# MaxInGaussian/SCFGP

Measured on AMD Instinct MI355X. Metric: NLML+grad evals/sec, higher is better.
Workload: dtype f32

## Files before the change

scfgp_amd/csrc/gram.hip:

```cpp
#include "kernels.h"
#include "tile_cfgs.h"

#include <algorithm>

#ifdef SCFGP_TRACE
constexpr int TRACE_CAP = 1 << 16;
__device__ unsigned long long g_trace[TRACE_CAP][4];
#define TRACE_BEGIN() const unsigned long long tr_t0 = __builtin_amdgcn_s_memrealtime()
#define TRACE_END(kind)                                                                                     \
    do {                                                                                                    \
        __syncthreads();                                                                                    \
        if (threadIdx.x == 0 && j < TRACE_CAP) {                                                            \
            g_trace[j][0] = tr_t0; g_trace[j][1] = __builtin_amdgcn_s_memrealtime();                        \
            g_trace[j][2] = (unsigned long long)__builtin_amdgcn_s_getreg((20 << 0) | (0 << 6) | (3 << 11)) |             \
                            ((unsigned long long)__builtin_amdgcn_s_getreg((4 << 0) | (0 << 6) | (31 << 11)) << 8);       \
            g_trace[j][3] = (unsigned long long)(kind);                                                     \
        }                                                                                                   \
    } while (0)
int64_t trace_read(void* host, int64_t max_bytes) {
    const int64_t n = max_bytes < (int64_t)sizeof(g_trace) ? max_bytes : (int64_t)sizeof(g_trace);
    return hipMemcpyFromSymbol(host, HIP_SYMBOL(g_trace), n) == hipSuccess ? n : -2;
}
#else
#define TRACE_BEGIN()
// ... 69 lines not shown
    double* __restrict__ slab, double* __restrict__ slab_hi, char* smem_raw) {
    if (diag) gram_body_impl<Cfg, WEIGHT, STRIP, true>(Phi, ld, w, side, r0, r1, chunk, acol, bcol, sideout, slab, slab_hi, smem_raw);
    else gram_body_impl<Cfg, WEIGHT, STRIP, false>(Phi, ld, w, side, r0, r1, chunk, acol, bcol, sideout, slab, slab_hi, smem_raw);
}

struct GramDma {
    static constexpr int BM = 256, BN = 128, A_BYTES = 16 * BM * 4, B_BYTES = 16 * BN * 4, W_OFF = A_BYTES + B_BYTES,
                         STAGE = W_OFF + 256, STAGES = 3, LDS_BYTES = STAGES * STAGE, DMA_PER_WAVE = (A_BYTES + B_BYTES) / 1024 / 8;
    static_assert(DMA_PER_WAVE == 3, "8 waves, 24 KiB of operands per stage");
};
typedef __attribute__((address_space(3))) void lds_void;
typedef const __attribute__((address_space(1))) void gbl_void;
__device__ __forceinline__ lds_void* lds_ptr(const char* p) { return (lds_void*)(uintptr_t)((unsigned)(uintptr_t)p); }
struct GramDmaWide {
    static constexpr int BM = 64, BN = 512, A_BYTES = 16 * BM * 4, B_BYTES = 16 * BN * 4, W_OFF = A_BYTES + B_BYTES,
                         STAGE = W_OFF + 256, STAGES = 2, LDS_BYTES = STAGES * STAGE, NINSTR = (A_BYTES + B_BYTES) / 1024, DMA_PER_WAVE = 5;
    static_assert(NINSTR == 36 && 2 * LDS_BYTES <= 160 * 1024, "two workgroups per CU");
};
struct GramDmaSq {
    static constexpr int BM = 128, BN = 128, A_BYTES = 16 * BM * 4, B_BYTES = 16 * BN * 4, W_OFF = A_BYTES + B_BYTES,
                         STAGE = W_OFF + 256, STAGES = 3, LDS_BYTES = STAGES * STAGE, DMA_PER_WAVE = (A_BYTES + B_BYTES) / 1024 / 8;
    static_assert(DMA_PER_WAVE == 2, "8 waves, 16 KiB of operands per stage");
};
struct GramDmaPair {
    static constexpr int BM = 256, BN = 128, A_BYTES = 16 * BM * 4, B_BYTES = 0, W_OFF = A_BYTES,
                         STAGE = W_OFF + 256, STAGES = 3, LDS_BYTES = STAGES * STAGE, DMA_PER_WAVE = A_BYTES / 1024 / 8;
    static_assert(DMA_PER_WAVE == 2, "8 waves, 16 KiB of operands per stage");
};
template <class D, bool WEIGHT, bool DIAG, bool TRANS = false>
__device__ __forceinline__ void gram_pipe_dma(
    const float* __restrict__ Phi, int64_t ld, const float* __restrict__ ws2,
    int64_t r0, int64_t r1, int64_t chunk, int acol, int bcol, double* __restrict__ sideout,
    double* __restrict__ slab, double* __restrict__ slab_hi, char* smem) {
    constexpr bool WIDE = D::BM == 64, SQ = D::BM == 128, PAIR = D::B_BYTES == 0;
    constexpr int RING = D::STAGES, TM = SQ ? 2 : 4;
    typedef std::integral_constant<int, 0> H0;
    typedef std::integral_constant<int, 1> H1;
    constexpr bool WS = WEIGHT || DIAG;
    constexpr int DPW = D::DMA_PER_WAVE, NRD = 4 + (WEIGHT || DIAG ? 2 : 0), NM = 8 * TM, PRE = 2;
    static_assert(PRE + DPW + 1 + NRD <= NM, "one fetch or read per MFMA behind the barrier");
    static_assert(!(PAIR && DIAG), "the paired diagonal blocks carry no side sums");
    static_assert(!TRANS || (D::BM == 256 && D::B_BYTES != 0 && !DIAG), "transposed flush: off-diagonal tall tiles");
    int tid = threadIdx.x;
    asm volatile("" : "+v"(tid));
    const int lane = tid & 63, wave = __builtin_amdgcn_readfirstlane(tid >> 6), i = lane & 15, q = lane >> 4;
    const int wm0 = WIDE ? 0 : (wave >> 1) * (16 * TM), wn0 = WIDE ? wave * 64 : (wave & 1) * 64;
    const char* src[DPW]; int dst[DPW];
#pragma unroll
    for (int u = 0; u < DPW; ++u) {
        const int t = WIDE ? wave + 8 * u : DPW * wave + u;
        const float* g;
        if constexpr (PAIR) g = Phi + (r0 + t) * ld + (lane < 32 ? acol : bcol - 128) + 4 * lane;
        else if constexpr (SQ) g = t < 8 ? Phi + (r0 + 2 * t + (lane >> 5)) * ld + acol + ((4 * (lane & 31) - 32 * (lane >> 5)) & 127)
                                    : Phi + (r0 + 2 * (t - 8) + (lane >> 5)) * ld + bcol + 4 * (lane & 31);
        else if constexpr (WIDE) g = t < 4 ? Phi + (r0 + 4 * t + (lane >> 4)) * ld + acol + 4 * (lane & 15) : Phi + (r0 + ((t - 4) >> 1)) * ld + bcol + 256 * ((t - 4) & 1) + 4 * lane;
        else g = t < 16 ? Phi + (r0 + t) * ld + acol + 4 * lane : Phi + (r0 + 2 * (t - 16) + (lane >> 5)) * ld + bcol + 4 * (lane & 31);
        src[u] = reinterpret_cast<const char*>(g);
        dst[u] = t * 1024;
    }
    const bool last_u = !WIDE || wave < 4;
    const int64_t step = 16 * ld * (int64_t)sizeof(float);
    const char* wsrc = WS ? reinterpret_cast<const char*>(ws2 + 2 * r0) + 4 * lane : nullptr;
    const bool ws_wave = WS && wave == 0;
    const auto fetch_one = [&](auto uc, int slot) {
        constexpr int u = decltype(uc)::value;
        char* base = smem + slot * D::STAGE;
        if constexpr (u < DPW) {
            if (u < DPW - 1 || last_u) {
                __builtin_amdgcn_global_load_lds((gbl_void*)src[u], lds_ptr(base + dst[u]), 16, 0, 0);
                src[u] += step;
            }
        } else if (ws_wave) {
            __builtin_amdgcn_global_load_lds((gbl_void*)wsrc, lds_ptr(base + D::W_OFF), 4, 0, 0);
            wsrc += 128;
        }
    };
    const int ring = (int)(uintptr_t)smem;
    const int pa0 = SQ ? ring + q * (D::BM * 4) + ((wm0 + 2 * i + 32 * (q & 1)) & 127) * 4 : ring + q * (D::BM * 4) + (wm0 + 4 * i) * 4, pb0 = PAIR ? ring + q * (D::BM * 4) + ((wm0 & 128) + wn0 + 4 * i) * 4 : ring + D::A_BYTES + q * (D::BN * 4) + (wn0 + 4 * i) * 4, pw0 = ring + D::W_OFF + q * 8;
    typedef float v2f __attribute__((ext_vector_type(2)));
    typedef float afrag_t __attribute__((ext_vector_type(TM)));
    afrag_t fa[2][2]; v4f fb[2][2];
    v2f fws[2][2];
    v4f acc[TM][4];
    afrag_t sacc = 0.f;
    const auto read_one = [&](auto hc, auto rc, int stage) {
        constexpr int h = decltype(hc)::value, R = decltype(rc)::value, kk = 2 * h + (R & 1);
        (void)&fws; (void)&pw0; (void)&fa; (void)&fb; (void)&pa0; (void)&pb0;
        if constexpr (R < 2 && SQ) asm volatile("ds_read_b64 %0, %1 offset:%2" : "=v"(fa[h][R & 1]) : "v"(stage + pa0), "n"(kk * 4 * D::BM * 4));
        else if constexpr (R < 2) asm volatile("ds_read_b128 %0, %1 offset:%2" : "=v"(fa[h][R & 1]) : "v"(stage + pa0), "n"(kk * 4 * D::BM * 4));
        else if constexpr (R < 4) asm volatile("ds_read_b128 %0, %1 offset:%2" : "=v"(fb[h][R & 1]) : "v"(stage + pb0), "n"(kk * 4 * (PAIR ? D::BM : D::BN) * 4));
        else asm volatile("ds_read_b64 %0, %1 offset:%2" : "=v"(fws[h][R & 1]) : "v"(stage + pw0), "n"(kk * 32));
    };
#define SCFGP_WAIT_FRAGS(what, h)                                                                                                        \
    do {                                                                                                                                 \
        if constexpr (WS)                                                                                                                \
            asm volatile("s_waitcnt " what : "+v"(fa[h][0]), "+v"(fa[h][1]), "+v"(fb[h][0]), "+v"(fb[h][1]), "+v"(fws[h][0]), "+v"(fws[h][1]) :: "memory"); \
        else asm volatile("s_waitcnt " what : "+v"(fa[h][0]), "+v"(fa[h][1]), "+v"(fb[h][0]), "+v"(fb[h][1]) :: "memory");              \
        __builtin_amdgcn_sched_barrier(0);                                                                                               \
        if constexpr (DIAG) { sacc += fws[h][0][1] * fa[h][0]; sacc += fws[h][1][1] * fa[h][1]; }        \
        if constexpr (WEIGHT) { fa[h][0] *= fws[h][0][0]; fa[h][1] *= fws[h][1][0]; }                                                    \
        __builtin_amdgcn_sched_barrier(0);                                                                                               \
    } while (0)
    const auto mfma_one = [&](auto hc, auto ic) {
        constexpr int h = decltype(hc)::value, I = decltype(ic)::value, k2 = I / (4 * TM), tm = I / 4 % TM, tn = I % 4;
        acc[tm][tn] = __builtin_amdgcn_mfma_f32_16x16x4f32(fa[h][k2][tm], fb[h][k2][tn], acc[tm][tn], 0, 0, 0);
        __builtin_amdgcn_sched_barrier(0);
    };
    const auto second_half_pre = [&]() { static_for<PRE>([&](auto ic) { mfma_one(H1(), ic); }); };
    const auto second_half = [&](auto fc, auto rdc, int fslot, int next) {
        static_for<NM - PRE>([&](auto ic) {
            constexpr int I = decltype(ic)::value;
            mfma_one(H1(), std::integral_constant<int, I + PRE>());
            if constexpr (I < DPW + 1) {
                if constexpr (decltype(fc)::value && (I < DPW || WS)) { fetch_one(ic, fslot); __builtin_amdgcn_sched_barrier(0); }
            } else if constexpr (I - DPW - 1 < NRD) {
                if constexpr (decltype(rdc)::value) { read_one(H0(), std::integral_constant<int, I - DPW - 1>(), next); __builtin_amdgcn_sched_barrier(0); }
            }
        });
    };
    const auto first_half = [&](int next) {
        static_for<NM>([&](auto ic) {
            mfma_one(H0(), ic);
            if constexpr (decltype(ic)::value < NRD) { read_one(H1(), ic, next); __builtin_amdgcn_sched_barrier(0); }
        });
    };
    double* sl = TRANS ? (wm0 >= 128 ? slab_hi : slab) + (int64_t)wn0 * 128 + (wm0 & 127)
               : WIDE  ? slab + (int64_t)(wn0 >> 7) * (128 * 128) + (wn0 & 127)
                       : (wm0 >= 128 ? slab_hi + (int64_t)(wm0 - 128) * 128 : slab + (int64_t)wm0 * 128) + wn0;
    bool first = true;
    const auto flush = [&]() {
        int lf = lane;
        asm volatile("" : "+v"(lf));
        const int i = lf & 15, q = lf >> 4;
        if constexpr (TRANS) {
#pragma unroll
            for (int tn = 0; tn < 4; ++tn)
#pragma unroll
                for (int r = 0; r < 4; ++r) {
                    v4d* d = reinterpret_cast<v4d*>(sl + (4 * i + tn) * 128 + 4 * (4 * q + r));
                    const v4d v = v4d{(double)acc[0][tn][r], (double)acc[1][tn][r], (double)acc[2][tn][r], (double)acc[3][tn][r]};
                    *d = first ? v : *d + v;
                }
        } else {
#pragma unroll
        for (int tm = 0; tm < TM; ++tm)
#pragma unroll
            for (int r = 0; r < 4; ++r) {
                v4d* d = reinterpret_cast<v4d*>(sl + (TM * (4 * q + r) + tm) * 128 + 4 * i);
                const v4d v = v4d{(double)acc[tm][0][r], (double)acc[tm][1][r], (double)acc[tm][2][r], (double)acc[tm][3][r]};
                *d = first ? v : *d + v;
            }
        }
        if constexpr (DIAG) {
#pragma unroll
            for (int tm = 0; tm < TM; ++tm) {
                double x = (double)sacc[tm];
                x += __shfl_xor(x, 16); x += __shfl_xor(x, 32);
                if (q == 0 && wn0 == 0) { double* d = sideout + wm0 + TM * i + tm; *d = first ? x : *d + x; }
            }
            sacc = 0.f;
        }
#pragma unroll
        for (int tm = 0; tm < TM; ++tm)
#pragma unroll
            for (int tn = 0; tn < 4; ++tn) acc[tm][tn] = v4f{0.f, 0.f, 0.f, 0.f};
        first = false;
    };
#pragma unroll
    for (int tm = 0; tm < TM; ++tm)
#pragma unroll
        for (int tn = 0; tn < 4; ++tn) acc[tm][tn] = v4f{0.f, 0.f, 0.f, 0.f};
    const auto strip_rest = [&]() {
        if constexpr (WIDE)
            for (int e = tid; e < 4 * 64 * 128; e += 512) slab[(e / (64 * 128)) * (128 * 128) + 64 * 128 + e % (64 * 128)] = 0.0;
    };
    const int nst = (int)((r1 - r0) / 16), per_chunk = (int)(chunk / 16);
    if (nst == 0) { flush(); strip_rest(); return; }
    static_for<DPW + 1>([&](auto uc) { fetch_one(uc, 0); });
    if (RING == 3 && nst > 1) static_for<DPW + 1>([&](auto uc) { fetch_one(uc, 1); });
    const auto wait_landed = [&](bool more) {
        if (RING == 3 && more) {
            if (ws_wave) asm volatile("s_waitcnt vmcnt(%0)" :: "n"(DPW + 1) : "memory"); else asm volatile("s_waitcnt vmcnt(%0)" :: "n"(DPW) : "memory");
        }
        else asm volatile("s_waitcnt vmcnt(0)" ::: "memory");
    };
    const auto next_slot = [&](int sl_) { return sl_ == RING - 1 ? 0 : sl_ + 1; };
    int slot = 0, s = 0;
    while (s < nst) {
        const int cend = s + per_chunk < nst ? s + per_chunk : nst;
        wait_landed(s + 1 < nst);
        __builtin_amdgcn_s_barrier();
        asm volatile("" ::: "memory");
        if (s + RING - 1 < nst) { const int fslot = slot == 0 ? RING - 1 : slot - 1; static_for<DPW + 1>([&](auto uc) { fetch_one(uc, fslot); }); }
        static_for<NRD>([&](auto rc) { read_one(H0(), rc, slot * D::STAGE); });
        static_for<NRD>([&](auto rc) { read_one(H1(), rc, slot * D::STAGE); });
        SCFGP_WAIT_FRAGS("lgkmcnt(0)", 0);
        static_for<NM>([&](auto ic) { mfma_one(H0(), ic); });
// ... 103 lines not shown
        slot ^= 1;
    }
#pragma unroll
    for (int tm = 0; tm < 2; ++tm)
#pragma unroll
        for (int r = 0; r < 4; ++r) {
            double* d = slab + (wm0 + 2 * (q + 4 * r) + tm) * D::B + wn0 + 2 * i;
            *reinterpret_cast<v2d*>(d) = v2d{acc[tm][0][r], acc[tm][1][r]};
            *reinterpret_cast<v2d*>(d + 32) = v2d{acc[tm][2][r], acc[tm][3][r]};
        }
    if constexpr (DIAG) {
#pragma unroll
        for (int tm = 0; tm < 2; ++tm) {
            double x = sacc[tm];
            x += __shfl_xor(x, 16); x += __shfl_xor(x, 32);
            if (q == 0 && wn0 == 0) sideout[wm0 + 2 * i + tm] = x;
        }
    }
}

template <bool BIG> __host__ __device__ inline int gram_jobs_per_split(int nfull, int nstrip) {
    if (!BIG) return nfull * (nfull + 1) / 2 + nstrip * (nfull + 1);
    const int R = nfull / 2, odd = nfull & 1, nsb = nstrip * (nfull + 1);
    return R * R + nsb / 4 + (R + 1) / 2 + odd * (R + 1) + nsb % 4;
}
template <class Cfg, class SCfg, class BCfg, bool WEIGHT, bool BIG>
__device__ __forceinline__ void gram_job(
    const int j, const typename Cfg::T* __restrict__ Phi, int64_t ld, const double* __restrict__ w, const double* __restrict__ side,
    const float* __restrict__ ws2, const RowSplits& rs, int64_t chunk, int nfull, int nstrip, double* __restrict__ sidepart,
    double* __restrict__ slabs, char* smem_raw) {
    static_assert(Cfg::THREADS == SCfg::THREADS && Cfg::THREADS == BCfg::THREADS && Cfg::THREADS == 512 &&
                  Cfg::BN == SCfg::BN && Cfg::BN == BCfg::BN && Cfg::BM == Cfg::BN && GramDmaWide::BM == SCfg::BM && GramDmaWide::BN == 4 * Cfg::BN,
                  "one launch, five tile shapes");
    TRACE_BEGIN();
    constexpr int B = Cfg::BN;
    const int nall = nfull + nstrip, ntile_all = nall * (nall + 1) / 2;
    const int per_split = gram_jobs_per_split<BIG>(nfull, nstrip);
    const int split = j / per_split;
    int u = j % per_split, acol, bcol, slab_t, slab_t2 = 0, kind = 0;
    bool diag = false;
    const auto tri = [](int ti, int tj) { return ti * (ti + 1) / 2 + tj; };
    if (BIG) {
        const int R = nfull / 2, Rp = (R + 1) / 2, nbig = R * R, nsmall = Rp + (nfull & 1) * (R + 1), nwide = nstrip * (nfull + 1) / 4;
        if (u < nbig) {
            int a = (int)sqrtf((float)u);
            while ((a + 1) * (a + 1) <= u) ++a;
            while (a * a > u) --a;
            const int b = u - a * a;
            acol = 2 * a * B; bcol = b * B; slab_t = tri(2 * a, b); slab_t2 = tri(2 * a + 1, b); kind = 2;
            diag = side != nullptr && b == 2 * a;
        } else if (u < nbig + nwide) {
            const int q = u - nbig;
            acol = nfull * B; bcol = 4 * q * B; slab_t = tri(nfull, 4 * q); kind = 3;
            diag = side != nullptr && nfull >= 4 * q && nfull < 4 * q + 4;
        } else if (u < nbig + nwide + Rp) {
            const int m = u - nbig - nwide, i = 2 * (2 * m) + 1;
            acol = bcol = i * B; slab_t = tri(i, i);
            if (2 * m + 1 < R) { const int i2 = 2 * (2 * m + 1) + 1; bcol = i2 * B; slab_t2 = tri(i2, i2); kind = 4; }
        } else if (u < nbig + nwide + nsmall) {
            const int i = nfull - 1, b = u - nbig - nwide - Rp;
            if (b < R) { acol = 2 * b * B; bcol = i * B; slab_t = tri(i, 2 * b); slab_t2 = tri(i, 2 * b + 1); kind = 5; }
            else { acol = bcol = i * B; slab_t = tri(i, i); diag = side != nullptr; }
        } else {
            const int tj = 4 * nwide + u - nbig - nwide - nsmall;
            acol = nfull * B; bcol = tj * B; slab_t = tri(nfull, tj); kind = 1; diag = side != nullptr && tj == nfull;
        }
    } else {
        const int noff = nfull * (nfull - 1) / 2;
        if (u < nfull) {
            acol = bcol = u * B; slab_t = tri(u, u); diag = side != nullptr;
        } else if (u < nfull + noff) {
            u -= nfull;
            int tq = (int)((sqrtf(8.0f * u + 1.0f) - 1.0f) * 0.5f);
            while ((tq + 1) * (tq + 2) / 2 <= u) ++tq;
            while (tq * (tq + 1) / 2 > u) --tq;
            const int ti = tq + 1, tj = u - tq * (tq + 1) / 2;
            acol = ti * B; bcol = tj * B; slab_t = tri(ti, tj);
        } else {
            const int tj = u - nfull - noff;
            acol = nfull * B; bcol = tj * B; slab_t = tri(nfull, tj); kind = 1; diag = side != nullptr && tj == nfull;
        }
    }
    int64_t r0, r1;
    rs.range(split, r0, r1);
    double* slab = slabs + ((int64_t)split * ntile_all + slab_t) * (B * B);
    double* slab2 = slabs + ((int64_t)split * ntile_all + slab_t2) * (B * B);
    double* sideout = sidepart + (int64_t)split * ld + acol;
    if (kind == 1) { gram_body<SCfg, WEIGHT, true>(Phi, ld, w, side, r0, r1, chunk, acol, bcol, diag, sideout, slab, nullptr, smem_raw); TRACE_END(kind); return; }
    if constexpr (BIG) {
        if (kind == 2) {
            if (diag) gram_pipe_dma<GramDma, WEIGHT, true>(Phi, ld, ws2, r0, r1, chunk, acol, bcol, sideout, slab, slab2, smem_raw);
            else gram_pipe_dma<GramDma, WEIGHT, false>(Phi, ld, ws2, r0, r1, chunk, acol, bcol, sideout, slab, slab2, smem_raw);
            TRACE_END(kind); return;
        }
        if (kind == 5) {
            gram_pipe_dma<GramDma, WEIGHT, false, true>(Phi, ld, ws2, r0, r1, chunk, acol, bcol, sideout, slab, slab2, smem_raw);
            TRACE_END(kind); return;
        }
        if (kind == 4) {
            gram_pipe_dma<GramDmaPair, WEIGHT, false>(Phi, ld, ws2, r0, r1, chunk, acol, bcol, sideout, slab, slab2, smem_raw);
            TRACE_END(kind); return;
        }
        if (kind == 0) {
            if (diag) gram_pipe_dma<GramDmaSq, WEIGHT, true>(Phi, ld, ws2, r0, r1, chunk, acol, bcol, sideout, slab, nullptr, smem_raw);
            else gram_pipe_dma<GramDmaSq, WEIGHT, false>(Phi, ld, ws2, r0, r1, chunk, acol, bcol, sideout, slab, nullptr, smem_raw);
            TRACE_END(kind); return;
        }
        if (kind == 3) {
            if (diag) gram_pipe_dma<GramDmaWide, WEIGHT, true>(Phi, ld, ws2, r0, r1, chunk, acol, bcol, sideout, slab, nullptr, smem_raw);
            else gram_pipe_dma<GramDmaWide, WEIGHT, false>(Phi, ld, ws2, r0, r1, chunk, acol, bcol, sideout, slab, nullptr, smem_raw);
            TRACE_END(kind); return;
        }
    }
    if constexpr (!BIG && sizeof(typename Cfg::T) == 8) {
        if (diag) gram_sq_dma64<WEIGHT, true>(Phi, ld, w, side, r0, r1, acol, bcol, sideout, slab, smem_raw);
        else gram_sq_dma64<WEIGHT, false>(Phi, ld, w, side, r0, r1, acol, bcol, sideout, slab, smem_raw);
    } else
        gram_body<Cfg, WEIGHT, false>(Phi, ld, w, side, r0, r1, chunk, acol, bcol, diag, sideout, slab, nullptr, smem_raw);
    TRACE_END(kind);
}

template <class Cfg, class SCfg, class BCfg, bool WEIGHT, bool BIG>
__global__ __launch_bounds__(Cfg::THREADS)
__attribute__((amdgpu_waves_per_eu(4, 4)))
void gram_kernel(
    const typename Cfg::T* __restrict__ Phi, int64_t ld, const double* __restrict__ w, const double* __restrict__ side,
    const float* __restrict__ ws2, RowSplits rs, int64_t chunk, int nfull, int nstrip, double* __restrict__ sidepart,
    double* __restrict__ slabs, int njobs, int* __restrict__ head) {
    SMEM_DECL;
    if ((int)gridDim.x >= njobs) {
        gram_job<Cfg, SCfg, BCfg, WEIGHT, BIG>((int)xcd_remap(blockIdx.x, gridDim.x), Phi, ld, w, side, ws2, rs, chunk, nfull, nstrip, sidepart, slabs, smem_raw);
        return;
    }
    __shared__ int s_job;
    const int q8 = njobs / 8, r8 = njobs % 8;
// ... 55 lines not shown
                run(lb);
            } else {
                ZbarLoader<S, T, Cfg::BN, Cfg::BK, Cfg::LDB, Cfg::THREADS, NS> lb(Phi + c0 * ld, Pb + c0 * ld, ld, J, tj * Cfg::BN, threadIdx.x);
                run(lb);
            }
        }
        slab_flush<Cfg>(acc, slab, first);
        first = false;
    }
    if (Cfg::BM < 128)
        for (int e = threadIdx.x; e < (128 - Cfg::BM) * 128; e += Cfg::THREADS) slab[Cfg::BM * 128 + e] = 0.0;
}

static int num_cus() {
    static int n = 0;
    if (n == 0) {
        int dev = 0; hipDeviceProp_t prop;
        if (hipGetDevice(&dev) == hipSuccess && hipGetDeviceProperties(&prop, dev) == hipSuccess) n = prop.multiProcessorCount;
        if (n <= 0) n = 256;
    }
    return n;
}
template <typename T>
int GramKernels<T>::gram_jobs(const Geom& g) { return gram_jobs_per_split<sizeof(T) == 4>(g.gfull, g.gstrip); }

RowSplits gram_row_splits(int jobs, int64_t Np, bool f32, int nsplit_override, int taper) {
    int64_t s = ((f32 ? 4224 : 6144) + jobs - 1) / jobs;
    s = std::max<int64_t>(s, 56);
    const int64_t smax = std::max<int64_t>(Np / (f32 ? 3072 : 2048), 1);
    if (s > smax) s = smax;
    int gran = 256;
    if (jobs * s < 256 && Np / 64 > s) { gran = 64; s = std::min<int64_t>(Np / 64, (512 + jobs - 1) / jobs); }
    if (nsplit_override > 0) s = std::min<int64_t>(nsplit_override, Np / gran);
    if (s < 1) s = 1;
    RowSplits rs;
    rs.gran = gran; rs.nrb = Np / gran;
    if (s >= 16) { rs.groups = 8; rs.units = (int)((s + 4) / 8); rs.taper = taper && rs.units >= 5 ? (taper == 1 ? 3 : taper + 2) : 0; }
    else { rs.groups = 1; rs.units = (int)s; rs.taper = 0; }
    rs.nsplit = rs.groups * rs.per_group();
    return rs;
}

__global__ __launch_bounds__(256) void gram_pack_ws(const double* __restrict__ w, const double* __restrict__ side, float* __restrict__ ws2, int64_t Np) {
    typedef float v2f __attribute__((ext_vector_type(2)));
    for (int64_t n = (int64_t)blockIdx.x * 256 + threadIdx.x; n < Np; n += (int64_t)gridDim.x * 256)
        reinterpret_cast<v2f*>(ws2)[n] = v2f{w ? (float)w[n] : 1.f, side ? (float)side[n] : 0.f};
}
template <typename T>
void GramKernels<T>::gram(const Geom& g, const T* Phi, const double* w, const double* side, const RowSplits& rs, int64_t chunk,
                          double* slabs, double* sidepart, int* qhead, float* ws2, hipStream_t st) {
    typedef typename GramCfg<T, 128>::type Cfg;
    typedef typename GramStripCfg<T>::type SCfg;
    typedef typename GramBigCfg<T>::type BCfg;
    constexpr bool BIG = sizeof(T) == 4;
    const int njobs = gram_jobs(g) * rs.nsplit;
    if (chunk <= 0 || chunk > g.Np) chunk = g.Np;
    chunk = round_up(chunk, 256);
    constexpr int L0 = Cfg::LDS_BYTES > SCfg::LDS_BYTES ? Cfg::LDS_BYTES : SCfg::LDS_BYTES;
    constexpr int L1 = !BIG && GramDma64::LDS_BYTES > L0 ? GramDma64::LDS_BYTES : L0;
    constexpr int L2 = BIG && GramDma::LDS_BYTES > L1 ? GramDma::LDS_BYTES : L1;
    constexpr int LDS = BIG && GramDmaWide::LDS_BYTES > L2 ? GramDmaWide::LDS_BYTES : L2;
    static_assert(2 * LDS <= 160 * 1024, "two workgroups per CU");
    const int resident = 2 * num_cus();
    const bool persistent = njobs >= 6 * resident;
    if (persistent) (void)hipMemsetAsync(qhead, 0, sizeof(int) * 8, st);
    if (BIG && (w || side)) hipLaunchKernelGGL(gram_pack_ws, dim3((unsigned)std::min<int64_t>((g.Np + 255) / 256, 2048)), dim3(256), 0, st, w, side, ws2, g.Np);
    const auto launch = [&](auto kernel) {
        allow_big_lds(kernel, LDS);
#ifdef SCFGP_GRAM_LD0
        const int64_t ld = 0;
#else
        const int64_t ld = g.Kp;
#endif
        hipLaunchKernelGGL(kernel, dim3(persistent ? resident : njobs), dim3(Cfg::THREADS), LDS, st, Phi, ld, w, side, (const float*)ws2, rs, chunk,
                           g.gfull, g.gstrip, sidepart, slabs, njobs, qhead);
    };
    if (w) launch(gram_kernel<Cfg, SCfg, BCfg, true, BIG>);
    else launch(gram_kernel<Cfg, SCfg, BCfg, false, BIG>);
}

template <typename T, bool PLAIN>
static void tn_product(const double* A, int Dp, const T* Bsrc, const T* Bsrc2, int64_t ldb, int J, int64_t Np, int nsplit, int64_t chunk,
                       double* slabs, hipStream_t st) {
    const int ntm = (Dp + 127) / 128, ntn = (J + 127) / 128;
// ... 47 lines not shown
__global__ void rsel_kernel(const double* __restrict__ params, int D, int S, int M, T* __restrict__ out, int Kp, int ncol) {
    const int64_t total = (int64_t)Kp * ncol;
    const double* rF = params + 3 + (int64_t)D * S;
    for (int64_t i = (int64_t)blockIdx.x * 256 + threadIdx.x; i < total; i += (int64_t)gridDim.x * 256) {
        const int k = (int)(i / ncol), c = (int)(i % ncol);
        T v = 0;
        if (c < S) { if (k < S) v = k == c ? (T)1 : (T)0; else if (k < S + M) v = (T)rF[(int64_t)(k - S) * S + c]; }
        out[(int64_t)k * Kp + c] = v;
    }
}
template <typename T>
void GramKernels<T>::rsel(const Geom& g, const double* params, T* out, hipStream_t st) {
    hipLaunchKernelGGL(rsel_kernel<T>, dim3(1024), dim3(256), 0, st, params, g.D, g.S, g.M, out, g.Kp, (int)round_up(g.S, 64));
}
template <typename T>
void GramKernels<T>::xtz(const Geom& g, const double* Xt, const T* Phi, const T* Phibar, int nsplit, int64_t chunk, double* slabs,
                          hipStream_t st) {
    tn_product<T, false>(Xt, g.Dp, Phi, Phibar, (int64_t)g.Kp, g.J, g.Np, nsplit, chunk, slabs, st);
}
template struct GramKernels<double>;
template struct GramKernels<float>;

__global__ __launch_bounds__(256) void reduce_tri_kernel(const double* __restrict__ slabs, int nsplit, int ntiles, int B,
                                                         double* __restrict__ packed) {
    const int t = blockIdx.x;
    for (int e = 2 * (blockIdx.y * 256 + threadIdx.x); e < B * B; e += 2 * gridDim.y * 256) {
        const double* src = slabs + (int64_t)t * (B * B) + e;
        const int64_t step = (int64_t)ntiles * (B * B);
        v2d s = v2d{0, 0};
        int sp = 0;
        for (; sp + 8 <= nsplit; sp += 8) {
            v2d x[8];
#pragma unroll
            for (int u = 0; u < 8; ++u) x[u] = *reinterpret_cast<const v2d*>(src + (sp + u) * step);
#pragma unroll
            for (int u = 0; u < 8; ++u) s += x[u];
        }
        for (; sp < nsplit; ++sp) s += *reinterpret_cast<const v2d*>(src + sp * step);
        *reinterpret_cast<v2d*>(packed + (int64_t)t * B * B + e) = s;
    }
}
void reduce_tri_tiles(const double* slabs, int nsplit, int nts, int tile, double* packed, hipStream_t st) {
    const int ntiles = nts * (nts + 1) / 2;
    hipLaunchKernelGGL(reduce_tri_kernel, dim3(ntiles, 16), dim3(256), 0, st, slabs, nsplit, ntiles, tile, packed);
}
__global__ __launch_bounds__(1024) void reduce_side_kernel(const double* __restrict__ sidepart, int nsplit, int Kp, int ncov, double* __restrict__ vec) {
    __shared__ double run[16][64];
    const int j = blockIdx.x * 64 + (threadIdx.x & 63), sub = threadIdx.x >> 6;
    double s = 0;
    if (j < ncov)
        for (int sp = sub; sp < nsplit; sp += 16) s += sidepart[(int64_t)sp * Kp + j];
    run[sub][threadIdx.x & 63] = s;
    __syncthreads();
    if (sub == 0 && j < Kp) {
#pragma unroll
        for (int k = 1; k < 16; ++k) s += run[k][threadIdx.x];
        vec[j] = s;
    }
}
void reduce_side(const double* sidepart, int nsplit, int Kp, int ncov, double* vec, hipStream_t st) {
    hipLaunchKernelGGL(reduce_side_kernel, dim3((Kp + 63) / 64), dim3(1024), 0, st, sidepart, nsplit, Kp, ncov, vec);
}
__global__ __launch_bounds__(256) void unpack_tri_kernel(const double* __restrict__ packed, int B, double* __restrict__ full, int64_t ld) {
    const int t = blockIdx.x;
    int ti = (int)((sqrtf(8.0f * t + 1.0f) - 1.0f) * 0.5f);
    while ((ti + 1) * (ti + 2) / 2 <= t) ++ti;
    while (ti * (ti + 1) / 2 > t) --ti;
// ... 26 lines not shown
```

scfgp_amd/csrc/kernels.h:

```cpp
#pragma once
#include "common.h"

struct Geom {
    int D, S, M, J, K, P;
    int Dp;
    int Jp;
    int Sp;
    int lowrank;
    int Kp;
    int tile;
    int gfull;
    int gstrip;
    int64_t N;
    int64_t Np;
};

struct RowSplits {
    int nsplit;
    int groups;
    int units;
    int taper;
    int gran;
    int64_t nrb;
    __host__ __device__ int per_group() const { return units + taper; }
// ... 9 lines not shown
            e0 = base + den - (den >> k);
            e1 = k == taper ? base + den : base + den - (den >> (k + 1));
        }
        r0 = (g0 + len * e0 / (den * units)) * gran;
        r1 = (g0 + len * e1 / (den * units)) * gran;
    }
};
RowSplits gram_row_splits(int jobs_per_split, int64_t Np, bool f32, int nsplit_override, int taper);

struct Projection { const double* Fall; const double* Lall; const double* Rall; double* Tt; };

template <typename T>
struct FmapKernels {
    static void featuremap(const Geom& g, const double* Xt, const Projection& pr, const Scal* sc, T* Phi, hipStream_t st);
    static void convert(const double* src, T* dst, int K, int Kp, hipStream_t st);
    static void convert_transposed(const double* src, T* dst, int K, int Kp, hipStream_t st);
};

template <typename T>
struct GramKernels {
    static void gram(const Geom& g, const T* Phi, const double* w, const double* side, const RowSplits& rs, int64_t chunk,
                     double* slabs, double* sidepart, int* qhead, float* ws2, hipStream_t st);
    static int gram_jobs(const Geom& g);
    static void xtz(const Geom& g, const double* Xt, const T* Phi, const T* Phibar, int nsplit, int64_t chunk, double* slabs,
                    hipStream_t st);
    static void zbar_inplace(const Geom& g, const T* Phi, T* Phibar, hipStream_t st);
    static void rsel(const Geom& g, const double* params, T* out, hipStream_t st);
    static void tn_plain(const double* A, int Dp, const T* Bm, int64_t ldb, int J, int64_t Np, int nsplit, int64_t chunk, double* slabs,
                         hipStream_t st);
};

struct F16Operands { const unsigned* Phi16; const char* B16; const float* scale; unsigned* V16; const float* vbound; };

template <typename T>
struct ApplyKernels {
    static void apply_v(const Geom& g, const T* Phi, const T* Bm, T* V, double* vpart, const double* alpha, double* mupart,
                        hipStream_t st, int dma = 0, const F16Operands* f16 = nullptr);
    static void apply_predict(const Geom& g, const T* Phi, const T* LiT, double* vpart, const double* alpha, double* mupart,
                              hipStream_t st);
    static void apply_c(const Geom& g, const T* Phi, const T* LiT, const T* Li, T* C, double* vpart, const double* alpha,
                        const double* beta, double* mupart, hipStream_t st, int dma = 0);
    static void apply_vc(const Geom& g, const T* C, const T* Li, const T* LiT, T* V, hipStream_t st, int dma = 0);
    static void apply_phibar(const Geom& g, const T* Phi, const T* Abar, T* V, const double* p, const double* q,
                             const double* y, const double* alpha, const double* ut, hipStream_t st, int dma = 0, const F16Operands* f16 = nullptr);
    static void apply_plain(const Geom& g, const T* A, const T* Bm, T* Out, int Kc, int ncols, hipStream_t st);
    static void rowstats(const Geom& g, const double* mupart, const double* vpart, const double* y,
// ... 7 lines not shown
    template <int EPI, int BN>
    static int apply(const Geom& g, int njt, int col0, int slot0, const float* Phi, const F16Operands& f, float* V,
                     double* vpart, const double* p, const double* q, const double* y, const double* alpha, const double* ut, double* mu,
                     hipStream_t st, int64_t rb0, int64_t nrb);
    static bool apply_runs(const Geom& g);
    static constexpr size_t F16_PAD = 1024;
    static int side_blocks(const Geom& g);
    static void split_phi(const Geom& g, const float* Phi, const double* y, const Scal* sc, unsigned* Phi16, double* sidepart, float* tmp,
                          hipStream_t st);
    static void v_bound(const Geom& g, const double* B, const Scal* sc, float* tmp, hipStream_t st);
    static void split_v(const Geom& g, const float* V, const double* q, const double* p, unsigned* V16g, unsigned* qV16g, double* sidepart,
                        float* tmp, hipStream_t st);
    static int gram_chunks(const Geom& g, int64_t chunk);
    static int gram_tiles(const Geom& g);
    static void gram(const Geom& g, const unsigned* A16g, const unsigned* B16g, const float* scale, int64_t chunk, double* slabs, hipStream_t st);
};

template <typename T> struct SweepKernels : FmapKernels<T>, GramKernels<T>, ApplyKernels<T> {};

int64_t trace_read(void* host, int64_t max_bytes);
int64_t apply_trace_read(void* host, int64_t max_bytes);
int64_t chol_trace_read(void* host, int64_t max_bytes);

void reduce_tri_tiles(const double* slabs, int nsplit, int nts, int tile, double* packed, hipStream_t st);
void unpack_tri_tiles(const double* packed, int nts, int tile, double* full, int64_t ld, hipStream_t st);
void reduce_full_tiles(const double* slabs, int nsplit, int ntm, int ntn, double* out, int64_t ldo, hipStream_t st);
void reduce_side(const double* sidepart, int nsplit, int Kp, int ncov, double* vec, hipStream_t st);
void reduce_scalars(double* partial, int nblocks, int width, double* scalars, int slot0, hipStream_t st);
void sum_squares(const double* y, int64_t n, double* scalars, int slot, double* scratch, hipStream_t st);

void unpack_params(const Geom& g, const double* params, double* F, double* Fall, double* Lall, double* Rall, Scal* sc, hipStream_t st);
void grad_epilogue(const Geom& g, const double* params, const double* F, const double* XZ, int64_t ldxz,
                   double* work, double* scalars, int64_t Nglobal, double* grad, hipStream_t st,
                   const double* TZ = nullptr, int64_t ldtz = 0, const double* XU = nullptr, int64_t ldxu = 0);
void finalize_cost(const Geom& g, const Scal* sc, double* scalars, const double* yy, const double* t2kb,
                   int64_t Nglobal, double* grad, int want_grad, hipStream_t st);
void write_status(double* xs, double ran1, double cap1, double cap2, double fail, hipStream_t st);
void pack_data(const Geom& g, const double* Xraw, const double* yraw, const int64_t* idx, double* Xt, double* y, hipStream_t st,
               int mode = 0, const double* sp = nullptr);
void pad_square(const double* src, int K, int Kp, double* dst, hipStream_t st);

constexpr int YPOST_BLOCKS = 64;
void ypost_mean(const double* ys, int64_t n, double* out, hipStream_t st);
void ypost_chunk(double* mu, double* sd, const double* ys, int64_t n, int mode, const double* sp, const double* ymean,
                 double* part, hipStream_t st);
void ypost_metrics(const double* part, int nparts, int64_t n, double* out, hipStream_t st);

// ... 35 lines not shown
```

scfgp_amd/csrc/scfgp_api.hip:

```cpp
#include "../../include/scfgp_hip.h"
#include "kernels.h"

#include <dlfcn.h>
#if __has_include(<rccl/rccl.h>)
#include <rccl/rccl.h>
#else
extern "C" {
typedef struct ncclComm* ncclComm_t;
typedef struct { char internal[128]; } ncclUniqueId;
typedef enum { ncclSuccess = 0 } ncclResult_t;
typedef enum { ncclFloat64 = 8 } ncclDataType_t;
typedef enum { ncclSum = 0 } ncclRedOp_t;
ncclResult_t ncclGetUniqueId(ncclUniqueId*);
ncclResult_t ncclCommInitRank(ncclComm_t*, int, ncclUniqueId, int);
ncclResult_t ncclAllReduce(const void*, void*, size_t, ncclDataType_t, ncclRedOp_t, ncclComm_t, hipStream_t);
ncclResult_t ncclCommDestroy(ncclComm_t);
const char* ncclGetErrorString(ncclResult_t);
}
#endif

#include <algorithm>
#include <cmath>
#include <cstdlib>
#include <cstring>
// ... 425 lines not shown
template <typename T> struct Impl {
    typedef SweepKernels<T> SK;
    static void gram_to(scfgp_ctx* c, const T* Mx, const double* w, const double* side, double* out, const char* name) {
        const Geom& g = c->g;
        const int nts = g.Kp / g.tile, ntiles = nts * (nts + 1) / 2;
        if constexpr (sizeof(T) == 4) {
            if (c->f16_gram()) {
                const int nch = F16x3Kernels::gram_chunks(g, c->f16_chunk());
                { ProfScope ps(c, w ? "split_v" : "split_phi");
                  if (w) F16x3Kernels::split_v(g, (const float*)Mx, w, side, F16x3Kernels::apply_runs(g) ? nullptr : c->d_V16g, c->d_qV16g,
                                               c->d_f16side, c->d_f16tmp, c->st);
                  else F16x3Kernels::split_phi(g, (const float*)Mx, side, c->d_sc, c->d_Phi16, c->d_f16side, c->d_f16tmp, c->st); }
                { ProfScope ps(c, name);
                  F16x3Kernels::gram(g, w ? c->d_V16g : c->d_Phi16, w ? c->d_qV16g : c->d_Phi16, c->d_f16tmp + 4, c->f16_chunk(), c->d_slabs, c->st); }
                { ProfScope ps(c, "reduce_tiles"); reduce_tri_tiles(c->d_slabs, nch, nts, g.tile, out, c->st);
                  reduce_side(c->d_f16side, F16x3Kernels::side_blocks(g), g.Kp, g.gfull * g.tile + g.gstrip * 64, out + c->n_pk, c->st); }
                return;
            }
        }
        const int gs = c->splits.nsplit;
        double* sidepart = c->d_slabs + (size_t)gs * ntiles * g.tile * g.tile;
        { ProfScope ps(c, name);
          SK::gram(g, Mx, w, side, c->splits, c->dtype == SCFGP_F32 ? c->gram_chunk : 0, c->d_slabs, sidepart, c->d_flag + 8, c->d_ws2, c->st); }
        { ProfScope ps(c, "reduce_tiles"); reduce_tri_tiles(c->d_slabs, gs, nts, g.tile, out, c->st);
          reduce_side(sidepart, gs, g.Kp, g.gfull * g.tile + g.gstrip * 64, out + c->n_pk, c->st); }
    }
    static int pass1(scfgp_ctx* c) {
        const Geom& g = c->g;
        if (!c->in_train) HIPCHK(c, hipMemsetAsync(c->d_flag, 0, sizeof(int) * 4, c->st));
        const bool use64 = sizeof(T) == 4 && c->use64();
        c->last_cform = c->want_cform();
        if ((use64 && c->phi64_cap < g.Np) || (c->last_cform && c->c_cap < g.Np)) {
            c->err = "pass1: auxiliary row buffer missing"; return SCFGP_EARG;
        }
        const Projection proj{c->d_Fall, c->d_Lall, c->d_Rall, c->d_Tt};
        if constexpr (sizeof(T) == 4) {
            if (use64) {
                typedef SweepKernels<double> SK64;
                const int nts = g.Kp / g.tile, ntiles = nts * (nts + 1) / 2, gs = c->splits64.nsplit;
                double* sidepart = c->d_slabs + (size_t)gs * ntiles * g.tile * g.tile;
                { ProfScope ps(c, "featuremap64"); SK64::featuremap(g, c->d_Xt, proj, c->d_sc, (double*)c->d_Phi64, c->st); }
                { ProfScope ps(c, "gram64");
                  SK64::gram(g, (const double*)c->d_Phi64, nullptr, c->d_y, c->splits64, 0, c->d_slabs, sidepart, c->d_flag + 8, nullptr, c->st); }
                { ProfScope ps(c, "reduce_tiles"); reduce_tri_tiles(c->d_slabs, gs, nts, g.tile, c->d_xp1, c->st);
                  reduce_side(sidepart, gs, g.Kp, g.gfull * g.tile + g.gstrip * 64, c->d_xp1 + c->n_pk, c->st); }
            }
        }
// ... 1064 lines not shown
```

Measured before the change: 4.916.

## Fold diagonal Gram blocks to compute only lower triangle, mirror in reduction

```diff
diff --git a/scfgp_amd/csrc/gram.hip b/scfgp_amd/csrc/gram.hip
--- a/scfgp_amd/csrc/gram.hip
+++ b/scfgp_amd/csrc/gram.hip
@@ -115,35 +115,47 @@
                          STAGE = W_OFF + 256, STAGES = 3, LDS_BYTES = STAGES * STAGE, DMA_PER_WAVE = (A_BYTES + B_BYTES) / 1024 / 8;
     static_assert(DMA_PER_WAVE == 2, "8 waves, 16 KiB of operands per stage");
 };
-struct GramDmaPair {
+struct GramDmaFold {
     static constexpr int BM = 256, BN = 128, A_BYTES = 16 * BM * 4, B_BYTES = 0, W_OFF = A_BYTES,
                          STAGE = W_OFF + 256, STAGES = 3, LDS_BYTES = STAGES * STAGE, DMA_PER_WAVE = A_BYTES / 1024 / 8;
     static_assert(DMA_PER_WAVE == 2, "8 waves, 16 KiB of operands per stage");
+};
+struct GramDmaDiag8 {
+    static constexpr int BM = 512, BN = 64, A_BYTES = 16 * BM * 4, B_BYTES = 0, W_OFF = A_BYTES,
+                         STAGE = W_OFF + 256, STAGES = 2, LDS_BYTES = STAGES * STAGE, DMA_PER_WAVE = A_BYTES / 1024 / 8;
+    static_assert(DMA_PER_WAVE == 4 && 2 * LDS_BYTES <= 160 * 1024, "8 waves, 32 KiB of operands per stage; two workgroups per CU");
 };
 template <class D, bool WEIGHT, bool DIAG, bool TRANS = false>
 __device__ __forceinline__ void gram_pipe_dma(
     const float* __restrict__ Phi, int64_t ld, const float* __restrict__ ws2,
     int64_t r0, int64_t r1, int64_t chunk, int acol, int bcol, double* __restrict__ sideout,
     double* __restrict__ slab, double* __restrict__ slab_hi, char* smem) {
-    constexpr bool WIDE = D::BM == 64, SQ = D::BM == 128, PAIR = D::B_BYTES == 0;
+    constexpr bool FOLD = std::is_same<D, GramDmaFold>::value, DIAG8 = std::is_same<D, GramDmaDiag8>::value;
+    constexpr bool WIDE = D::BM == 64, SQ = D::BM == 128, AIMG = D::B_BYTES == 0;
     constexpr int RING = D::STAGES, TM = SQ ? 2 : 4;
     typedef std::integral_constant<int, 0> H0;
     typedef std::integral_constant<int, 1> H1;
     constexpr bool WS = WEIGHT || DIAG;
     constexpr int DPW = D::DMA_PER_WAVE, NRD = 4 + (WEIGHT || DIAG ? 2 : 0), NM = 8 * TM, PRE = 2;
     static_assert(PRE + DPW + 1 + NRD <= NM, "one fetch or read per MFMA behind the barrier");
-    static_assert(!(PAIR && DIAG), "the paired diagonal blocks carry no side sums");
+    static_assert(!(DIAG8 && DIAG), "the diagonal quadrants carry no side sums");
     static_assert(!TRANS || (D::BM == 256 && D::B_BYTES != 0 && !DIAG), "transposed flush: off-diagonal tall tiles");
     int tid = threadIdx.x;
     asm volatile("" : "+v"(tid));
     const int lane = tid & 63, wave = __builtin_amdgcn_readfirstlane(tid >> 6), i = lane & 15, q = lane >> 4;
-    const int wm0 = WIDE ? 0 : (wave >> 1) * (16 * TM), wn0 = WIDE ? wave * 64 : (wave & 1) * 64;
+    const int wm0 = WIDE ? 0 : FOLD ? 64 * (wave < 4 ? wave : 2 + (wave & 1)) : DIAG8 ? 64 * wave : (wave >> 1) * (16 * TM);
+    const int wn0 = WIDE ? wave * 64 : FOLD ? (wave < 4 ? 0 : 64 + 64 * ((wave - 4) >> 1)) : DIAG8 ? 64 * wave : (wave & 1) * 64;
+    const int nown = DIAG8 ? bcol : 8;
     const char* src[DPW]; int dst[DPW];
 #pragma unroll
     for (int u = 0; u < DPW; ++u) {
         const int t = WIDE ? wave + 8 * u : DPW * wave + u;
         const float* g;
-        if constexpr (PAIR) g = Phi + (r0 + t) * ld + (lane < 32 ? acol : bcol - 128) + 4 * lane;
+        if constexpr (FOLD) g = Phi + (r0 + t) * ld + acol + 4 * lane;
+        else if constexpr (DIAG8) {
+            const int slot = 4 * (t & 1) + (lane >> 4);
+            g = Phi + (r0 + (t >> 1)) * ld + acol + (slot < nown ? slot : 0) * 128 + 64 + 4 * (lane & 15);
+        }
         else if constexpr (SQ) g = t < 8 ? Phi + (r0 + 2 * t + (lane >> 5)) * ld + acol + ((4 * (lane & 31) - 32 * (lane >> 5)) & 127)
                                     : Phi + (r0 + 2 * (t - 8) + (lane >> 5)) * ld + bcol + 4 * (lane & 31);
         else if constexpr (WIDE) g = t < 4 ? Phi + (r0 + 4 * t + (lane >> 4)) * ld + acol + 4 * (lane & 15) : Phi + (r0 + ((t - 4) >> 1)) * ld + bcol + 256 * ((t - 4) & 1) + 4 * lane;
@@ -169,7 +181,7 @@
         }
     };
     const int ring = (int)(uintptr_t)smem;
-    const int pa0 = SQ ? ring + q * (D::BM * 4) + ((wm0 + 2 * i + 32 * (q & 1)) & 127) * 4 : ring + q * (D::BM * 4) + (wm0 + 4 * i) * 4, pb0 = PAIR ? ring + q * (D::BM * 4) + ((wm0 & 128) + wn0 + 4 * i) * 4 : ring + D::A_BYTES + q * (D::BN * 4) + (wn0 + 4 * i) * 4, pw0 = ring + D::W_OFF + q * 8;
+    const int pa0 = SQ ? ring + q * (D::BM * 4) + ((wm0 + 2 * i + 32 * (q & 1)) & 127) * 4 : ring + q * (D::BM * 4) + (wm0 + 4 * i) * 4, pb0 = AIMG ? ring + q * (D::BM * 4) + (wn0 + 4 * i) * 4 : ring + D::A_BYTES + q * (D::BN * 4) + (wn0 + 4 * i) * 4, pw0 = ring + D::W_OFF + q * 8;
     typedef float v2f __attribute__((ext_vector_type(2)));
     typedef float afrag_t __attribute__((ext_vector_type(TM)));
     afrag_t fa[2][2]; v4f fb[2][2];
@@ -181,7 +193,7 @@
         (void)&fws; (void)&pw0; (void)&fa; (void)&fb; (void)&pa0; (void)&pb0;
         if constexpr (R < 2 && SQ) asm volatile("ds_read_b64 %0, %1 offset:%2" : "=v"(fa[h][R & 1]) : "v"(stage + pa0), "n"(kk * 4 * D::BM * 4));
         else if constexpr (R < 2) asm volatile("ds_read_b128 %0, %1 offset:%2" : "=v"(fa[h][R & 1]) : "v"(stage + pa0), "n"(kk * 4 * D::BM * 4));
-        else if constexpr (R < 4) asm volatile("ds_read_b128 %0, %1 offset:%2" : "=v"(fb[h][R & 1]) : "v"(stage + pb0), "n"(kk * 4 * (PAIR ? D::BM : D::BN) * 4));
+        else if constexpr (R < 4) asm volatile("ds_read_b128 %0, %1 offset:%2" : "=v"(fb[h][R & 1]) : "v"(stage + pb0), "n"(kk * 4 * (AIMG ? D::BM : D::BN) * 4));
         else asm volatile("ds_read_b64 %0, %1 offset:%2" : "=v"(fws[h][R & 1]) : "v"(stage + pw0), "n"(kk * 32));
     };
 #define SCFGP_WAIT_FRAGS(what, h)                                                                                                        \
@@ -217,7 +229,10 @@
             if constexpr (decltype(ic)::value < NRD) { read_one(H1(), ic, next); __builtin_amdgcn_sched_barrier(0); }
         });
     };
+    const int dblk = DIAG8 ? acol / 128 + wave : 0;
     double* sl = TRANS ? (wm0 >= 128 ? slab_hi : slab) + (int64_t)wn0 * 128 + (wm0 & 127)
+               : FOLD  ? (wm0 < 128 ? slab : wn0 < 128 ? slab_hi : slab_hi + 128 * 128) + (int64_t)(wm0 & 64) * 128 + (wn0 & 64)
+               : DIAG8 ? slab + (int64_t)(dblk * (dblk + 1) / 2 + dblk) * (128 * 128) + 64 * 128 + 64
                : WIDE  ? slab + (int64_t)(wn0 >> 7) * (128 * 128) + (wn0 & 127)
                        : (wm0 >= 128 ? slab_hi + (int64_t)(wm0 - 128) * 128 : slab + (int64_t)wm0 * 128) + wn0;
     bool first = true;
@@ -234,7 +249,7 @@
                     const v4d v = v4d{(double)acc[0][tn][r], (double)acc[1][tn][r], (double)acc[2][tn][r], (double)acc[3][tn][r]};
                     *d = first ? v : *d + v;
                 }
-        } else {
+        } else if (!DIAG8 || wave < nown) {
 #pragma unroll
         for (int tm = 0; tm < TM; ++tm)
 #pragma unroll
@@ -265,7 +280,10 @@
         for (int tn = 0; tn < 4; ++tn) acc[tm][tn] = v4f{0.f, 0.f, 0.f, 0.f};
     const auto strip_rest = [&]() {
         if constexpr (WIDE)
-            for (int e = tid; e < 4 * 64 * 128; e += 512) slab[(e / (64 * 128)) * (128 * 128) + 64 * 128 + e % (64 * 128)] = 0.0;
+            for (int k = 0; k < 4 * 64 * 128 / 512; ++k) {
+                const int e = 512 * k + tid;
+                slab[(e / (64 * 128)) * (128 * 128) + 64 * 128 + e % (64 * 128)] = 0.0;
+            }
     };
     const int nst = (int)((r1 - r0) / 16), per_chunk = (int)(chunk / 16);
     if (nst == 0) { flush(); strip_rest(); return; }
@@ -415,7 +433,13 @@
 template <bool BIG> __host__ __device__ inline int gram_jobs_per_split(int nfull, int nstrip) {
     if (!BIG) return nfull * (nfull + 1) / 2 + nstrip * (nfull + 1);
     const int R = nfull / 2, odd = nfull & 1, nsb = nstrip * (nfull + 1);
-    return R * R + nsb / 4 + (R + 1) / 2 + odd * (R + 1) + nsb % 4;
+    return R * (R - 1) + R + nsb / 4 + (R + 3) / 4 + odd * (R + 1) + nsb % 4;
+}
+template <class SCfg, bool WEIGHT>
+__device__ __attribute__((noinline)) void gram_strip_job(
+    const float* __restrict__ Phi, int64_t ld, const double* __restrict__ w, const double* __restrict__ side, int64_t r0, int64_t r1,
+    int64_t chunk, int acol, int bcol, bool diag, double* __restrict__ sideout, double* __restrict__ slab, char* smem_raw) {
+    gram_body<SCfg, WEIGHT, true>(Phi, ld, w, side, r0, r1, chunk, acol, bcol, diag, sideout, slab, nullptr, smem_raw);
 }
 template <class Cfg, class SCfg, class BCfg, bool WEIGHT, bool BIG>
 __device__ __forceinline__ void gram_job(
@@ -434,28 +458,30 @@
     bool diag = false;
     const auto tri = [](int ti, int tj) { return ti * (ti + 1) / 2 + tj; };
     if (BIG) {
-        const int R = nfull / 2, Rp = (R + 1) / 2, nbig = R * R, nsmall = Rp + (nfull & 1) * (R + 1), nwide = nstrip * (nfull + 1) / 4;
+        const int R = nfull / 2, nbig = R * (R - 1), nwide = nstrip * (nfull + 1) / 4, nd8 = (R + 3) / 4, nsmall = (nfull & 1) * (R + 1);
         if (u < nbig) {
-            int a = (int)sqrtf((float)u);
-            while ((a + 1) * (a + 1) <= u) ++a;
-            while (a * a > u) --a;
-            const int b = u - a * a;
+            int a = (int)((1.0f + sqrtf(1.0f + 4.0f * u)) * 0.5f);
+            while (a * (a + 1) <= u) ++a;
+            while (a * (a - 1) > u) --a;
+            const int b = u - a * (a - 1);
             acol = 2 * a * B; bcol = b * B; slab_t = tri(2 * a, b); slab_t2 = tri(2 * a + 1, b); kind = 2;
-            diag = side != nullptr && b == 2 * a;
-        } else if (u < nbig + nwide) {
-            const int q = u - nbig;
+        } else if (u < nbig + R) {
+            const int a = u - nbig;
+            acol = bcol = 2 * a * B; slab_t = tri(2 * a, 2 * a); slab_t2 = tri(2 * a + 1, 2 * a); kind = 6;
+            diag = side != nullptr;
+        } else if (u < nbig + R + nwide) {
+            const int q = u - nbig - R;
             acol = nfull * B; bcol = 4 * q * B; slab_t = tri(nfull, 4 * q); kind = 3;
             diag = side != nullptr && nfull >= 4 * q && nfull < 4 * q + 4;
-        } else if (u < nbig + nwide + Rp) {
-            const int m = u - nbig - nwide, i = 2 * (2 * m) + 1;
-            acol = bcol = i * B; slab_t = tri(i, i);
-            if (2 * m + 1 < R) { const int i2 = 2 * (2 * m + 1) + 1; bcol = i2 * B; slab_t2 = tri(i2, i2); kind = 4; }
-        } else if (u < nbig + nwide + nsmall) {
-            const int i = nfull - 1, b = u - nbig - nwide - Rp;
+        } else if (u < nbig + R + nwide + nd8) {
+            const int m = u - nbig - R - nwide;
+            acol = 8 * m * B; bcol = 2 * R - 8 * m < 8 ? 2 * R - 8 * m : 8; slab_t = 0; kind = 7;
+        } else if (u < nbig + R + nwide + nd8 + nsmall) {
+            const int i = nfull - 1, b = u - nbig - R - nwide - nd8;
             if (b < R) { acol = 2 * b * B; bcol = i * B; slab_t = tri(i, 2 * b); slab_t2 = tri(i, 2 * b + 1); kind = 5; }
             else { acol = bcol = i * B; slab_t = tri(i, i); diag = side != nullptr; }
         } else {
-            const int tj = 4 * nwide + u - nbig - nwide - nsmall;
+            const int tj = 4 * nwide + u - nbig - R - nwide - nd8 - nsmall;
             acol = nfull * B; bcol = tj * B; slab_t = tri(nfull, tj); kind = 1; diag = side != nullptr && tj == nfull;
         }
     } else {
@@ -479,19 +505,13 @@
     double* slab = slabs + ((int64_t)split * ntile_all + slab_t) * (B * B);
     double* slab2 = slabs + ((int64_t)split * ntile_all + slab_t2) * (B * B);
     double* sideout = sidepart + (int64_t)split * ld + acol;
-    if (kind == 1) { gram_body<SCfg, WEIGHT, true>(Phi, ld, w, side, r0, r1, chunk, acol, bcol, diag, sideout, slab, nullptr, smem_raw); TRACE_END(kind); return; }
     if constexpr (BIG) {
         if (kind == 2) {
-            if (diag) gram_pipe_dma<GramDma, WEIGHT, true>(Phi, ld, ws2, r0, r1, chunk, acol, bcol, sideout, slab, slab2, smem_raw);
-            else gram_pipe_dma<GramDma, WEIGHT, false>(Phi, ld, ws2, r0, r1, chunk, acol, bcol, sideout, slab, slab2, smem_raw);
+            gram_pipe_dma<GramDma, WEIGHT, false>(Phi, ld, ws2, r0, r1, chunk, acol, bcol, sideout, slab, slab2, smem_raw);
             TRACE_END(kind); return;
         }
         if (kind == 5) {
             gram_pipe_dma<GramDma, WEIGHT, false, true>(Phi, ld, ws2, r0, r1, chunk, acol, bcol, sideout, slab, slab2, smem_raw);
-            TRACE_END(kind); return;
-        }
-        if (kind == 4) {
-            gram_pipe_dma<GramDmaPair, WEIGHT, false>(Phi, ld, ws2, r0, r1, chunk, acol, bcol, sideout, slab, slab2, smem_raw);
             TRACE_END(kind); return;
         }
         if (kind == 0) {
@@ -504,6 +524,20 @@
             else gram_pipe_dma<GramDmaWide, WEIGHT, false>(Phi, ld, ws2, r0, r1, chunk, acol, bcol, sideout, slab, nullptr, smem_raw);
             TRACE_END(kind); return;
         }
+        if (kind == 6) {
+            if (diag) gram_pipe_dma<GramDmaFold, WEIGHT, true>(Phi, ld, ws2, r0, r1, chunk, acol, bcol, sideout, slab, slab2, smem_raw);
+            else gram_pipe_dma<GramDmaFold, WEIGHT, false>(Phi, ld, ws2, r0, r1, chunk, acol, bcol, sideout, slab, slab2, smem_raw);
+            TRACE_END(kind); return;
+        }
+        if (kind == 7) {
+            gram_pipe_dma<GramDmaDiag8, WEIGHT, false>(Phi, ld, ws2, r0, r1, chunk, acol, bcol, sideout, slab, nullptr, smem_raw);
+            TRACE_END(kind); return;
+        }
+    }
+    if (kind == 1) {
+        if constexpr (BIG) gram_strip_job<SCfg, WEIGHT>(Phi, ld, w, side, r0, r1, chunk, acol, bcol, diag, sideout, slab, smem_raw);
+        else gram_body<SCfg, WEIGHT, true>(Phi, ld, w, side, r0, r1, chunk, acol, bcol, diag, sideout, slab, nullptr, smem_raw);
+        TRACE_END(kind); return;
     }
     if constexpr (!BIG && sizeof(typename Cfg::T) == 8) {
         if (diag) gram_sq_dma64<WEIGHT, true>(Phi, ld, w, side, r0, r1, acol, bcol, sideout, slab, smem_raw);
@@ -605,7 +639,13 @@
     return n;
 }
 template <typename T>
-int GramKernels<T>::gram_jobs(const Geom& g) { return gram_jobs_per_split<sizeof(T) == 4>(g.gfull, g.gstrip); }
+int GramKernels<T>::gram_jobs(const Geom& g) {
+    if (sizeof(T) == 8) return gram_jobs_per_split<false>(g.gfull, g.gstrip);
+    const int R = g.gfull / 2, nsb = g.gstrip * (g.gfull + 1);
+    return R * R + nsb / 4 + (R + 1) / 2 + (g.gfull & 1) * (R + 1) + nsb % 4;
+}
+template <typename T>
+int GramKernels<T>::gram_mirror_tiles(const Geom& g) { return sizeof(T) == 4 ? 2 * (g.gfull / 2) : 0; }
 
 RowSplits gram_row_splits(int jobs, int64_t Np, bool f32, int nsplit_override, int taper) {
     int64_t s = ((f32 ? 4224 : 6144) + jobs - 1) / jobs;
@@ -636,13 +676,14 @@
     typedef typename GramStripCfg<T>::type SCfg;
     typedef typename GramBigCfg<T>::type BCfg;
     constexpr bool BIG = sizeof(T) == 4;
-    const int njobs = gram_jobs(g) * rs.nsplit;
+    const int njobs = gram_jobs_per_split<BIG>(g.gfull, g.gstrip) * rs.nsplit;
     if (chunk <= 0 || chunk > g.Np) chunk = g.Np;
     chunk = round_up(chunk, 256);
     constexpr int L0 = Cfg::LDS_BYTES > SCfg::LDS_BYTES ? Cfg::LDS_BYTES : SCfg::LDS_BYTES;
     constexpr int L1 = !BIG && GramDma64::LDS_BYTES > L0 ? GramDma64::LDS_BYTES : L0;
     constexpr int L2 = BIG && GramDma::LDS_BYTES > L1 ? GramDma::LDS_BYTES : L1;
-    constexpr int LDS = BIG && GramDmaWide::LDS_BYTES > L2 ? GramDmaWide::LDS_BYTES : L2;
+    constexpr int L3 = BIG && GramDmaDiag8::LDS_BYTES > L2 ? GramDmaDiag8::LDS_BYTES : L2;
+    constexpr int LDS = BIG && GramDmaWide::LDS_BYTES > L3 ? GramDmaWide::LDS_BYTES : L3;
     static_assert(2 * LDS <= 160 * 1024, "two workgroups per CU");
     const int resident = 2 * num_cus();
     const bool persistent = njobs >= 6 * resident;
@@ -736,9 +777,32 @@
 template struct GramKernels<float>;
 
 __global__ __launch_bounds__(256) void reduce_tri_kernel(const double* __restrict__ slabs, int nsplit, int ntiles, int B,
-                                                         double* __restrict__ packed) {
+                                                         double* __restrict__ packed, int nmirror) {
     const int t = blockIdx.x;
+    int ti = (int)((sqrtf(8.0f * t + 1.0f) - 1.0f) * 0.5f);
+    while ((ti + 1) * (ti + 2) / 2 <= t) ++ti;
+    while (ti * (ti + 1) / 2 > t) --ti;
+    const bool fold = ti < nmirror && t == ti * (ti + 3) / 2;
+    if (fold && blockIdx.y < 4) {
+        for (int e = blockIdx.y * 256 + threadIdx.x; e < 64 * 64; e += 4 * 256) {
+            const int r = e % 64, c = 64 + e / 64;
+            const double* src = slabs + (int64_t)t * (B * B) + c * B + r;
+            const int64_t step = (int64_t)ntiles * (B * B);
+            double s = 0;
+            int sp = 0;
+            for (; sp + 8 <= nsplit; sp += 8) {
+                double x[8];
+#pragma unroll
+                for (int u = 0; u < 8; ++u) x[u] = src[(sp + u) * step];
+#pragma unroll
+                for (int u = 0; u < 8; ++u) s += x[u];
+            }
+            for (; sp < nsplit; ++sp) s += src[sp * step];
+            packed[(int64_t)t * B * B + r * B + c] = s;
+        }
+    }
     for (int e = 2 * (blockIdx.y * 256 + threadIdx.x); e < B * B; e += 2 * gridDim.y * 256) {
+        if (fold && e / B < 64 && e % B >= 64) continue;
         const double* src = slabs + (int64_t)t * (B * B) + e;
         const int64_t step = (int64_t)ntiles * (B * B);
         v2d s = v2d{0, 0};
@@ -754,9 +818,9 @@
         *reinterpret_cast<v2d*>(packed + (int64_t)t * B * B + e) = s;
     }
 }
-void reduce_tri_tiles(const double* slabs, int nsplit, int nts, int tile, double* packed, hipStream_t st) {
+void reduce_tri_tiles(const double* slabs, int nsplit, int nts, int tile, double* packed, hipStream_t st, int nmirror) {
     const int ntiles = nts * (nts + 1) / 2;
-    hipLaunchKernelGGL(reduce_tri_kernel, dim3(ntiles, 16), dim3(256), 0, st, slabs, nsplit, ntiles, tile, packed);
+    hipLaunchKernelGGL(reduce_tri_kernel, dim3(ntiles, 16), dim3(256), 0, st, slabs, nsplit, ntiles, tile, packed, nmirror);
 }
 __global__ __launch_bounds__(1024) void reduce_side_kernel(const double* __restrict__ sidepart, int nsplit, int Kp, int ncov, double* __restrict__ vec) {
     __shared__ double run[16][64];
diff --git a/scfgp_amd/csrc/kernels.h b/scfgp_amd/csrc/kernels.h
--- a/scfgp_amd/csrc/kernels.h
+++ b/scfgp_amd/csrc/kernels.h
@@ -55,6 +55,7 @@
     static void gram(const Geom& g, const T* Phi, const double* w, const double* side, const RowSplits& rs, int64_t chunk,
                      double* slabs, double* sidepart, int* qhead, float* ws2, hipStream_t st);
     static int gram_jobs(const Geom& g);
+    static int gram_mirror_tiles(const Geom& g);
     static void xtz(const Geom& g, const double* Xt, const T* Phi, const T* Phibar, int nsplit, int64_t chunk, double* slabs,
                     hipStream_t st);
     static void zbar_inplace(const Geom& g, const T* Phi, T* Phibar, hipStream_t st);
@@ -108,7 +109,7 @@
 int64_t apply_trace_read(void* host, int64_t max_bytes);
 int64_t chol_trace_read(void* host, int64_t max_bytes);
 
-void reduce_tri_tiles(const double* slabs, int nsplit, int nts, int tile, double* packed, hipStream_t st);
+void reduce_tri_tiles(const double* slabs, int nsplit, int nts, int tile, double* packed, hipStream_t st, int nmirror = 0);
 void unpack_tri_tiles(const double* packed, int nts, int tile, double* full, int64_t ld, hipStream_t st);
 void reduce_full_tiles(const double* slabs, int nsplit, int ntm, int ntn, double* out, int64_t ldo, hipStream_t st);
 void reduce_side(const double* sidepart, int nsplit, int Kp, int ncov, double* vec, hipStream_t st);
diff --git a/scfgp_amd/csrc/scfgp_api.hip b/scfgp_amd/csrc/scfgp_api.hip
--- a/scfgp_amd/csrc/scfgp_api.hip
+++ b/scfgp_amd/csrc/scfgp_api.hip
@@ -471,7 +471,7 @@
         double* sidepart = c->d_slabs + (size_t)gs * ntiles * g.tile * g.tile;
         { ProfScope ps(c, name);
           SK::gram(g, Mx, w, side, c->splits, c->dtype == SCFGP_F32 ? c->gram_chunk : 0, c->d_slabs, sidepart, c->d_flag + 8, c->d_ws2, c->st); }
-        { ProfScope ps(c, "reduce_tiles"); reduce_tri_tiles(c->d_slabs, gs, nts, g.tile, out, c->st);
+        { ProfScope ps(c, "reduce_tiles"); reduce_tri_tiles(c->d_slabs, gs, nts, g.tile, out, c->st, SK::gram_mirror_tiles(g));
           reduce_side(sidepart, gs, g.Kp, g.gfull * g.tile + g.gstrip * 64, out + c->n_pk, c->st); }
     }
     static int pass1(scfgp_ctx* c) {
```

Measured after the change: 4.961 (median of 6 runs). About the same (+0.9%).
